# chanchanchan97/ICAFusion

Hardware: AMD Instinct MI355X
Metric: RGB/IR image-pairs/sec (two-stream forward + NMS) (higher is better)
Workload: dtype bf16

## Files before the change

icafusion_amd/csrc/cstream.hip:

```cpp
#include "conv_common.h"

namespace icaf {

constexpr int CS_C = 64, CS_TH = 8, CS_TW = 16, CS_HH = CS_TH + 2, CS_HWD = CS_TW + 2, CS_PITCH = 24;
constexpr int CS_NIDX = CS_HH * CS_PITCH;
constexpr int CS_PATCH = CS_NIDX * 128;
constexpr int CS_WBYTES = 9 * CS_C * 128;
constexpr int CS_W2BYTES = CS_C * 128;
constexpr int CS_SO = CS_C * 2 + 16;
constexpr int CS_STG = 128 * CS_SO;
constexpr int CS_LDS = CS_WBYTES + CS_W2BYTES + 2 * CS_PATCH + CS_STG;
static_assert(CS_LDS <= 160 * 1024, "LDS capacity");

struct CsGeom { int tiles_x, tiles_y, ntile; };

template <int DT, bool CHAIN>
__global__ __launch_bounds__(512) __attribute__((amdgpu_waves_per_eu(2, 2))) void cstream_kernel(const ConvP p, const CsGeom gm) {
    using E = Elem<DT>;
    static_assert(DT != ICAF_F32, "16-bit types");
    constexpr int RB = 128, NSTEP = 4, VEC = E::VEC;
    extern __shared__ __attribute__((aligned(1024))) unsigned char lds[];
    unsigned char* wbuf = lds;
    unsigned char* w2buf = lds + CS_WBYTES;
    unsigned char* patch0 = w2buf + CS_W2BYTES;
    unsigned char* stg = patch0 + 2 * CS_PATCH;

    const int tid = threadIdx.x, lane = tid & 63, l31 = lane & 31, hi = lane >> 5;
    const int wave = __builtin_amdgcn_readfirstlane(tid >> 6);
    const int g = blockIdx.z;
    const int wm = wave & 3, wn = wave >> 2;
    const int sy = wm >> 1, sx = wm & 1;

    const __amdgpu_buffer_rsrc_t xr = __builtin_amdgcn_make_buffer_rsrc(
        (void*)((const typename E::type*)p.x + g * p.x_gs), 0, p.x_bytes, 0x00020000);
    const __amdgpu_buffer_rsrc_t wr = __builtin_amdgcn_make_buffer_rsrc(
        (void*)((const typename E::type*)p.w + g * p.w_gs), 0, p.w_bytes, 0x00020000);
    constexpr unsigned OOB = 0x80000000u;

    {
        const int rsub = lane >> 3;
        for (int t = wave; t < 72; t += 8) {
            const int c = t >> 3, j = t & 7;
// ... 31 lines not shown
            const int hy = idx / CS_PITCH, hx = idx - hy * CS_PITCH;
            const int gy = y0 - 1 + hy, gx = x0 - 1 + hx;
            const bool ok = hx < CS_HWD && (unsigned)gy < (unsigned)p.H && (unsigned)gx < (unsigned)p.W;
            const unsigned voff = ok ? img_off + (unsigned)((gy * p.W + gx) * p.ldx) * E::BYTES + (unsigned)(cs << 4) : OOB;
            __builtin_amdgcn_raw_ptr_buffer_load_lds(xr, (lds_ptr_t)(dst + (j << 10)), 16, voff, 0, 0, 0);
        }
    };

    f32x4 bq[4], bq2[4];
    {
        const float* __restrict__ bias = p.bias ? p.bias + g * p.bias_gs : nullptr;
        const float* __restrict__ bias2 = (CHAIN && p.bias2) ? p.bias2 + g * p.bias2_gs : nullptr;
#pragma unroll
        for (int qd = 0; qd < 4; ++qd) {
            const int n = wn * 32 + 8 * qd + 4 * hi;
            const f32x4 t1 = *(const f32x4*)((bias && n < p.Cout) ? bias + n : (const float*)p.w);
            bq[qd] = (bias && n < p.Cout) ? t1 : f32x4{0.f, 0.f, 0.f, 0.f};
            const f32x4 t2 = *(const f32x4*)((bias2 && n < p.Cout2) ? bias2 + n : (const float*)p.w);
            bq2[qd] = (bias2 && n < p.Cout2) ? t2 : f32x4{0.f, 0.f, 0.f, 0.f};
        }
#pragma unroll
        for (int qd = 0; qd < 4; ++qd) asm volatile("" : "+v"(bq[qd]), "+v"(bq2[qd]));
    }
    const int fkey = (l31 >> 1) & 7;
    int foff[NSTEP];
#pragma unroll
    for (int s = 0; s < NSTEP; ++s) foff[s] = (wn * 32 + l31) * RB + (((2 * s + hi) ^ fkey) << 4);
    const int lpy = sy * 4 + (l31 >> 3), lpx = sx * 8 + (l31 & 7);
    const int lbase = lpy * CS_PITCH + lpx;
    const int srow = wm * 32 + l31;

    int t = t_lo + lb;
    if (t >= t_hi) { wait_vmcnt<0>(); return; }
    issue_patch(t, 0);

    typename E::type* __restrict__ yg = (typename E::type*)p.y + g * p.y_gs;
    const typename E::type* __restrict__ rg = p.res ? (const typename E::type*)p.res + g * p.res_gs : nullptr;
    typename E::type* __restrict__ y2g = CHAIN ? (typename E::type*)p.y2 + g * p.y2_gs : nullptr;
    const float alpha_acc = p.alpha_acc[g], alpha_res = p.alpha_res[g];

    auto row_to_m = [&](int r, int b, int y0, int x0) {
        const int st = r >> 5, q = r & 31;
        const int gy = y0 + (st >> 1) * 4 + (q >> 3), gx = x0 + (st & 1) * 8 + (q & 7);
        return (gy < p.Ho && gx < p.Wo) ? (b * p.Ho + gy) * p.Wo + gx : -1;
    };
    u32x4 rres[2] = {u32x4{0u, 0u, 0u, 0u}, u32x4{0u, 0u, 0u, 0u}};
    auto flush = [&](typename E::type* dst, int ldd, int cout, int b, int y0, int x0, bool rr) {
#pragma unroll
        for (int it = 0; it < 2; ++it) {
            const int idx = tid + it * 512, row = idx >> 3, cv = idx & 7;
            const int m = row_to_m(row, b, y0, x0), n = cv * VEC;
            if (m >= 0 && n < cout) {
                u32x4 sv = *(const u32x4*)(stg + row * CS_SO + cv * 16);
                if (rr) {
                    float v[VEC], r[VEC];
                    unpack16<DT>(sv, v);
                    unpack16<DT>(rres[it], r);
#pragma unroll
                    for (int j = 0; j < VEC; ++j) v[j] = __builtin_fmaf(alpha_res, r[j], v[j]);
                    sv = pack16<DT>(v);
                }
                *(u32x4*)(dst + (long long)m * ldd + n) = sv;
            }
        }
    };
    auto load_res = [&](int b, int y0, int x0) {
#pragma unroll
        for (int it = 0; it < 2; ++it) {
            const int idx = tid + it * 512, row = idx >> 3, cv = idx & 7;
            const int m = row_to_m(row, b, y0, x0);
            rres[it] = *(const u32x4*)(rg + (long long)(m < 0 ? 0 : m) * p.ldr + cv * VEC);
        }
    };
    auto stage = [&](const f32x16& acc, const f32x4 (&bv)[4], float scale) {
#pragma unroll
        for (int qd = 0; qd < 4; ++qd) {
            const int nl = wn * 32 + 8 * qd + 4 * hi;
            float v[4];
#pragma unroll
            for (int j = 0; j < 4; ++j) v[j] = acc[4 * qd + j] + bv[qd][j] + 0.0f;
            silu4_f(v, v);
#pragma unroll
            for (int j = 0; j < 4; ++j) v[j] *= scale;
            u32x2 pk;
            if constexpr (DT == ICAF_BF16) { pk[0] = pack2_bf16(v[0], v[1]); pk[1] = pack2_bf16(v[2], v[3]); }
            else { pk[0] = pack2_f16(v[0], v[1]); pk[1] = pack2_f16(v[2], v[3]); }
            *(u32x2*)(stg + srow * CS_SO + nl * E::BYTES) = pk;
        }
    };

    int cur = 0, pb = -1, py0 = 0, px0 = 0;
    while (true) {
        int b, y0, x0;
        decode(t, b, y0, x0);
        const int tn = t + wgx;
        wait_vmcnt<0>();
        asm volatile("s_waitcnt lgkmcnt(0)" ::: "memory");
        __builtin_amdgcn_s_barrier();
        if (pb >= 0) {
            if constexpr (CHAIN) flush(y2g, p.ldy2, p.Cout2, pb, py0, px0, false);
            else flush(yg, p.ldy, p.Cout, pb, py0, px0, rg != nullptr);
        }
        if (rg) load_res(b, y0, x0);
        if (tn < t_hi) issue_patch(tn, cur ^ 1);
        const unsigned char* patch = patch0 + cur * CS_PATCH;
        f32x16 acc;
#pragma unroll
        for (int r = 0; r < 16; ++r) acc[r] = 0.0f;
#pragma unroll
        for (int c = 0; c < 9; ++c) {
            const int ky = c / 3, kx = c - 3 * ky;
            const int idx = lbase + ky * CS_PITCH + kx;
            const unsigned char* pe = patch + (idx << 7);
            const int key = (idx >> 1) & 7;
#pragma unroll
            for (int s = 0; s < NSTEP; ++s) {
                const u32x4 fp = *(const u32x4*)(pe + (((2 * s + hi) ^ key) << 4));
                const u32x4 fw = *(const u32x4*)(wbuf + c * (CS_C * RB) + foff[s]);
                mma_step<DT>(acc, fw, fp);
            }
        }
        lds_barrier();
        stage(acc, bq, alpha_acc);
        pb = b; py0 = y0; px0 = x0;
        if constexpr (CHAIN) {
            lds_barrier();
            if (rg) { wait_vmcnt<0>(); }
#pragma unroll
            for (int it = 0; it < 2; ++it) {
                const int idx = tid + it * 512, row = idx >> 3, cv = idx & 7;
                const int m = row_to_m(row, b, y0, x0), n = cv * VEC;
                if (m >= 0 && n < p.Cout) {
                    u32x4 sv = *(const u32x4*)(stg + row * CS_SO + cv * 16);
                    if (rg) {
                        float v[VEC], r[VEC];
                        unpack16<DT>(sv, v);
                        unpack16<DT>(rres[it], r);
#pragma unroll
                        for (int j = 0; j < VEC; ++j) v[j] = __builtin_fmaf(alpha_res, r[j], v[j]);
                        sv = pack16<DT>(v);
                        *(u32x4*)(stg + row * CS_SO + cv * 16) = sv;
                    }
                    if (p.keep1) *(u32x4*)(yg + (long long)m * p.ldy + n) = sv;
                }
            }
            lds_barrier();
            f32x16 acc2;
#pragma unroll
            for (int r = 0; r < 16; ++r) acc2[r] = 0.0f;
#pragma unroll
            for (int s = 0; s < NSTEP; ++s) {
                const u32x4 fp2 = *(const u32x4*)(stg + srow * CS_SO + ((2 * s + hi) << 4));
                const u32x4 fw2 = *(const u32x4*)(w2buf + foff[s]);
                mma_step<DT>(acc2, fw2, fp2);
            }
            lds_barrier();
            stage(acc2, bq2, 1.0f);
        }
        if (tn >= t_hi) break;
        t = tn;
        cur ^= 1;
    }
    wait_vmcnt<0>();
    lds_barrier();
    if constexpr (CHAIN) flush(y2g, p.ldy2, p.Cout2, pb, py0, px0, false);
    else flush(yg, p.ldy, p.Cout, pb, py0, px0, rg != nullptr);
}

int cstream_check(const icaf_conv_args* a, const ConvP& p) {
    if (a->dtype == ICAF_F32 || a->out_dtype != a->dtype) return fail(ICAF_ERR_UNSUPPORTED, "cstream: 16-bit types, out dtype == dtype");
    if (a->kh != 3 || a->kw != 3 || a->sh != 1 || a->sw != 1 || a->ph != 1 || a->pw != 1) return fail(ICAF_ERR_UNSUPPORTED, "cstream: 3x3 / stride 1 / pad 1 layers");
    if (a->Cin != CS_C || a->Cout > CS_C || a->Cout % 8 || a->Kp != 9 * CS_C) return fail(ICAF_ERR_UNSUPPORTED, "cstream: built for 64 -> (<= 64) channels (Cin = %d, Cout = %d, Kp = %d)", a->Cin, a->Cout, a->Kp);
    if (a->act != ICAF_ACT_SILU || a->pre) return fail(ICAF_ERR_UNSUPPORTED, "cstream: SiLU layers without a pre-activation term");
    if (p.x_bytes == 0) return fail(ICAF_ERR_UNSUPPORTED, "cstream: operand exceeds the 2 GiB buffer-descriptor range");
    if (!p.vec_y || (a->res && !p.vec_r)) return fail(ICAF_ERR_UNSUPPORTED, "cstream: y / res must take 16-byte vectors");
    if (a->w2) {
        if (a->Cout2 > CS_C || a->Cout2 % 8 || a->Kp2 != CS_C || !p.vec_y2 || a->Cout != CS_C) return fail(ICAF_ERR_UNSUPPORTED, "cstream: chained 1x1 of 64 -> (<= 64) channels with Kp2 = 64");
        if (a->res && !a->chain_keep) return fail(ICAF_ERR_UNSUPPORTED, "cstream: a residual needs chain_keep");
        if (a->chain_keep && (a->alpha_acc[0] != 1.0f || a->alpha_acc[1] != 1.0f)) return fail(ICAF_ERR_UNSUPPORTED, "cstream: chain_keep with alpha_acc != 1");
    }
    return ICAF_OK;
}

template <int DT, bool CHAIN>
static int launch_cstream_cfg(const ConvP& p, int groups, hipStream_t s) {
    CsGeom gm;
    gm.tiles_x = (p.Wo + CS_TW - 1) / CS_TW;
    gm.tiles_y = (p.Ho + CS_TH - 1) / CS_TH;
    gm.ntile = p.B * gm.tiles_x * gm.tiles_y;
    int dev = 0, cus = 256;
    ICAF_HIP(hipGetDevice(&dev));
    ICAF_HIP(hipDeviceGetAttribute(&cus, hipDeviceAttributeMultiprocessorCount, dev));
    int grid = (cus / groups) & ~7;
    if (grid < 8) grid = 8;
    ICAF_LDS_OPTIN((cstream_kernel<DT, CHAIN>), CS_LDS);
    cstream_kernel<DT, CHAIN><<<dim3((unsigned)grid, 1, (unsigned)groups), dim3(512), CS_LDS, s>>>(p, gm);
    ICAF_LAUNCH_CHECK();
    return ICAF_OK;
}

int launch_cstream(const icaf_conv_args* a, const ConvP& p, hipStream_t s) {
    int st = cstream_check(a, p);
    if (st) return st;
    if (a->dtype == ICAF_BF16) return a->w2 ? launch_cstream_cfg<ICAF_BF16, true>(p, a->groups, s) : launch_cstream_cfg<ICAF_BF16, false>(p, a->groups, s);
    return a->w2 ? launch_cstream_cfg<ICAF_F16, true>(p, a->groups, s) : launch_cstream_cfg<ICAF_F16, false>(p, a->groups, s);
}

}
```

icafusion_amd/csrc/igemm.hip:

```cpp
#include "conv_common.h"

static_assert(sizeof(icaf_conv_args) == 312, "icaf_conv_args layout is mirrored by ctypes in icafusion_amd/_lib.py");
static_assert(sizeof(icaf_bneck_args) == 376, "icaf_bneck_args layout is mirrored by ctypes in icafusion_amd/_lib.py");

namespace icaf {

template <int DT, int ODT, int BM, int BN, int WM, int WN, int ACT, int RB, int NS, int MODE, bool PRE, bool CHAIN = false>
__global__ __launch_bounds__((BM / WM) * (BN / WN) * 64) void igemm_dma_kernel(const ConvP p) {
    using E = Elem<DT>;
    using L = TileLds<DT, ODT, BM, BN>;
    constexpr int VEC = E::VEC;
    constexpr int BK = RB / E::BYTES;
    constexpr int SPR = RB / 16;
    constexpr int RPI = 1024 / RB;
    constexpr int AI = BM / RPI, BI = BN / RPI;
    constexpr int NW = (BM / WM) * (BN / WN);
    constexpr int NA = AI / NW;
    constexpr int NBF = BI / NW, NBR = BI % NW;
    constexpr int NBMAX = NBF + (NBR ? 1 : 0);
    constexpr int TM = WM / 32, TN = WN / 32;
    constexpr int WAVES_M = BM / WM;
    constexpr int STAGE = (BM + BN) * RB;
    constexpr int NSTEP = RB / 32;
    static_assert(AI % NW == 0 && (NW == 4 || NW == 8), "tile shape");
// ... 348 lines not shown
int launch_ctile(const icaf_conv_args* a, const ConvP& p, int shape, hipStream_t s);
int launch_bneck(const icaf_conv_args* a, const ConvP& p, int shape, hipStream_t s);
const char* ctile_tag(int shape);
int stream_check(const icaf_conv_args* a, const ConvP& p, int shape);
int launch_stream(const icaf_conv_args* a, const ConvP& p, int shape, hipStream_t s);
const char* stream_tag(int shape);
int cstream_check(const icaf_conv_args* a, const ConvP& p);
int launch_cstream(const icaf_conv_args* a, const ConvP& p, hipStream_t s);
int cwide_check(const icaf_conv_args* a, const ConvP& p, int shape);
int launch_cwide(const icaf_conv_args* a, const ConvP& p, int shape, hipStream_t s);
const char* cwide_tag(int shape);
int wreg_check(const icaf_conv_args* a, const ConvP& p, int shape);
int launch_wreg(const icaf_conv_args* a, const ConvP& p, int shape, hipStream_t s);
const char* wreg_tag(int shape);

static int pick_tile(const icaf_conv_args* a, const ConvP& p) {
    const bool dma_ok = p.x_bytes != 0;
    if (a->tile > 40 && a->tile < 90) return a->tile;
    if (a->tile >= 1 && a->tile <= 34 && a->tile % 10 >= 1 && a->tile % 10 <= 4) {
        const int pipe = a->tile / 10;
        return (pipe != 1 && !dma_ok) ? a->tile % 10 + 10 : a->tile;
    }
    if (a->tile == 25 || a->tile == 26 || a->tile == 28 || a->tile == 29) return a->tile;
    if (a->x2) return 81;
    const bool f32 = a->dtype == ICAF_F32 || a->out_dtype == ICAF_F32;
    const int N = a->Cout;
    const long long M = p.M;
    auto blocks = [&](int t) { return ((M + kTiles[t - 1].bm - 1) / kTiles[t - 1].bm) * ((N + kTiles[t - 1].bn - 1) / kTiles[t - 1].bn) * a->groups; };
    int t;
    if (N > 64 && !f32) t = 1;
    else if (N > 32) t = 2;
    else t = 3;
    if (t == 1 && blocks(1) < 512 && blocks(2) > blocks(1)) t = 2;
    if (blocks(t) < 512 && blocks(4) > blocks(t)) t = 4;
    if (!dma_ok) return t + 10;
    const int eb = a->dtype == ICAF_F32 ? 4 : 2;
    if (a->w2) {
        const int c = a->Cout > a->Cout2 ? a->Cout : a->Cout2;
        const bool w128 = ((long long)a->Cin * eb) % 128 == 0;
        if (c <= 64) return w128 ? 22 : 2;
        return w128 ? 21 : 1;
    }
    if (a->pre) {
        if (t > 2) t = 2;
        return ((long long)a->Cin * eb) % 128 == 0 ? t + 20 : t;
    }
    return (long long)p.K * eb >= 256 ? t + 20 : t;
// ... 168 lines not shown
    p.Kp2 = a->Kp2; p.Cout2 = a->Cout2; p.ldy2 = a->ldy2; p.keep1 = a->chain_keep;
    p.vec_y2 = a->w2 && (a->ldy2 % vo == 0) && (((uintptr_t)a->y2 & 15) == 0) && ((a->y2_gs * yb) % 16 == 0);
    p.w2_bytes = a->w2 ? (unsigned)((((long long)a->Cout2 + 127) / 128 * 128) * a->Kp2 * eb) : 0;
}

int conv_prepare(const icaf_conv_args* a, ConvP& p) {
    int st = validate(a);
    if (st) return st;
    fill(a, p);
    return ICAF_OK;
}

}

using namespace icaf;

extern "C" int icaf_conv2d(const icaf_conv_args* a, icaf_stream_t s) {
    int st = validate(a);
    if (st) return st;
    ConvP p;
    fill(a, p);
    const int tile = pick_tile(a, p);
    hipStream_t hs = S(s);
    if (a->x2 && tile != 81 && tile != 82) return fail(ICAF_ERR_UNSUPPORTED, "icaf_conv2d: x2 (C3 tail) is built for launch configurations 81 / 82 only (tile %d)", tile);
    if (tile == 71) return launch_cstream(a, p, hs);
    if (tile > 80) return launch_cwide(a, p, tile - 80, hs);
    if (tile > 70) return fail(ICAF_ERR_ARG, "unknown tile id %d", tile);
    if (tile > 60) return launch_wreg(a, p, tile - 60, hs);
    if (tile > 50) return launch_stream(a, p, tile - 50, hs);
    if (tile > 40) return launch_ctile(a, p, tile - 40, hs);
    if (a->dtype == ICAF_BF16)
        return a->out_dtype == ICAF_F32 ? launch_tile<ICAF_BF16, ICAF_F32>(p, a->groups, tile, hs)
                                        : launch_tile<ICAF_BF16, ICAF_BF16>(p, a->groups, tile, hs);
    if (a->dtype == ICAF_F16)
        return a->out_dtype == ICAF_F32 ? launch_tile<ICAF_F16, ICAF_F32>(p, a->groups, tile, hs)
                                        : launch_tile<ICAF_F16, ICAF_F16>(p, a->groups, tile, hs);
    return launch_tile<ICAF_F32, ICAF_F32>(p, a->groups, tile, hs);
}

extern "C" int icaf_bottleneck(const icaf_bneck_args* b, icaf_stream_t s) {
    if (!b || !b->w1) return fail(ICAF_ERR_ARG, "icaf_bottleneck: null pointer");
    const icaf_conv_args* a = &b->conv;
    int st = validate(a);
    if (st) return st;
    const int eb = a->dtype == ICAF_F32 ? 4 : 2;
    if (b->Kp1 * eb != 128) return fail(ICAF_ERR_ARG, "icaf_bottleneck: the packed 1x1 weights must have 128-byte rows (Kp1 = %d)", b->Kp1);
    if (a->pre) return fail(ICAF_ERR_ARG, "icaf_bottleneck: no pre-activation term");
    if (a->x2) return fail(ICAF_ERR_ARG, "icaf_bottleneck: conv.x2 must be NULL (the block's cv2 half is icaf_bneck_args.x2)");
    if (a->x == a->y) return fail(ICAF_ERR_ARG, "icaf_bottleneck: in-place operation is not possible (neighbouring patches read x)");
    ConvP p;
    fill(a, p);
    p.w1 = b->w1; p.bias1 = b->bias1; p.w1_gs = b->w1_gs; p.bias1_gs = b->bias1_gs; p.Kp1 = b->Kp1;
    p.w1_bytes = (unsigned)((((long long)a->Cout + 127) / 128 * 128) * b->Kp1 * eb);
    p.x2 = b->x2; p.x2_gs = b->x2_gs; p.ldx2 = b->ldx2;
    return launch_bneck(a, p, b->shape, S(s));
}

extern "C" int icaf_conv2d_kernel_name(const icaf_conv_args* a, char* buf, int buf_len) {
    int st = validate(a);
    if (st) return st;
    ConvP p;
    fill(a, p);
    const int tile = pick_tile(a, p);
    if (a->x2 && tile != 81 && tile != 82) return fail(ICAF_ERR_UNSUPPORTED, "icaf_conv2d: x2 (C3 tail) is built for launch configurations 81 / 82 only (tile %d)", tile);
    static const char* dn[] = {"f32", "bf16", "f16"};
    if (tile == 71) {
        st = cstream_check(a, p);
        if (st) return st;
        snprintf(buf, buf_len, "cstream_%s_8x16n64", dn[a->dtype]);
        return ICAF_OK;
    }
    if (tile > 80) {
        st = cwide_check(a, p, tile - 80);
        if (st) return st;
        snprintf(buf, buf_len, "cwide_%s_%s", dn[a->dtype], cwide_tag(tile - 80));
        return ICAF_OK;
    }
    if (tile > 70) return fail(ICAF_ERR_ARG, "unknown tile id %d", tile);
    if (tile > 60) {
        st = wreg_check(a, p, tile - 60);
        if (st) return st;
        snprintf(buf, buf_len, "igemm_wreg_%s_%s", dn[a->dtype], wreg_tag(tile - 60));
        return ICAF_OK;
    }
    if (tile > 50) {
        st = stream_check(a, p, tile - 50);
        if (st) return st;
// ... 14 lines not shown
```

icafusion_amd/models/common.py:

```python
import math

import torch
import torch.nn as nn

from .. import ops
from ..options import OPT
from ..engine import ImageIn, Plan, concat_view, from_act, to_act

BN_EPS_DEFAULT = 1e-5


def autopad(k, p=None):
    if p is None:
        p = k // 2 if isinstance(k, int) else [v // 2 for v in k]
    return p


def _pair(v):
    return (v, v) if isinstance(v, int) else tuple(v)


def _module_dtype(m, fallback=torch.float32):
    forced = getattr(m, "compute_dtype", None)
    if forced is not None:
# ... 182 lines not shown
        ch = None
        if chain is not None:
            convs, twin_convs, y2 = chain[:3]
            keep = len(chain) > 3 and bool(chain[3])
            x2 = chain[4] if len(chain) > 4 else None
            n2 = sum(c.conv.out_channels for c in convs)

            def pack2():
                packs = []
                for row in ([convs] + ([twin_convs] if paired else [])):
                    ws, bs = zip(*(c.folded() for c in row))
                    w2p, kp2 = ops.pack_conv_weight(torch.cat(ws), plan.dtype)
                    packs.append((w2p, kp2, ops.pack_bias(torch.cat(bs), n2)))
                if not paired:
                    return packs[0]
                return (torch.stack([p[0] for p in packs]).contiguous(), packs[0][1], torch.stack([p[2] for p in packs]).contiguous())
            w2p, kp2, b2p = self._cached(("chain",) + key_tail + tuple(id(c) for c in convs), pack2)
            ch = dict(w=w2p, kp=kp2, bias=b2p, y=y2, cout=n2, keep=keep)
            if x2 is not None:
                ch["x2"] = x2
            if not keep:
                out = y2[..., :c2] if y2.shape[-1] >= c2 else plan.act(B, Ho, Wo, c2, pair=paired)
        plan.add(ops.conv2d(x, wp, kp, bp, out, kh, kw, sh, sw, ph, pw, c1, c2, self._act_code(), res=res,
                            name=f"conv{kh}x{kw}s{sh}" + (("+cv3" if ch.get("x2") is not None else "+1x1") if ch else ""), pre=pre_term, chain=ch,
                            pre_nearest=pre_nearest))
        return (out if ch["keep"] else y2) if ch else out

    fuse_stem2 = True

    def stem2_ok(self, plan, x, nxt, c3):
        k0, k1 = self.conv, getattr(nxt, "conv", None)
        if not (self.fuse_stem2 and self.fuse_stem and isinstance(x, ImageIn) and x.pair and isinstance(nxt, Conv)
                and plan.dtype in (torch.bfloat16, torch.float16) and (not x.u8 or x.c0 == 0)):
            return False
        _, _, H, W = x.shape
        return ((k0.kernel_size, k0.stride, _pair(k0.padding), k0.in_channels, k0.out_channels) == ((6, 6), (2, 2), (2, 2), 3, 32)
                and k0.groups == 1 and isinstance(self.act, nn.SiLU) and H % 2 == 0 and W % 2 == 0
                and (k1.kernel_size, k1.stride, _pair(k1.padding), k1.in_channels, k1.out_channels) == ((3, 3), (2, 2), (1, 1), 32, 64)
                and nxt.chain_ok(plan, c3) and 2 * c3.cv1.conv.out_channels == 64)

    def emit_stem2(self, plan, x, twin, nxt, nxt_twin, convs, twin_convs, y2):
        key_tail = (plan.dtype, plan.device, id(twin))

        def stack(packs):
            return (torch.stack([p[0] for p in packs]).contiguous(), packs[0][1], torch.stack([p[2] for p in packs]).contiguous())

        def pack_row(rows, transform, cin_pad):
# ... 14 lines not shown
        return y2

    chain_fuse = True

    def chain_ok(self, plan, c3):
        k, cv = self.conv, c3.cv1.conv
        n1, n2 = k.out_channels, 2 * cv.out_channels
        return (self.chain_fuse and plan.dtype in (torch.bfloat16, torch.float16) and isinstance(self.act, nn.SiLU)
                and hasattr(k, "kernel_size") and k.kernel_size == (3, 3) and k.groups == 1 and k.in_channels % 32 == 0
                and cv.kernel_size == (1, 1) and cv.stride == (1, 1) and cv.in_channels == n1
                and c3.cv2.conv.out_channels == cv.out_channels and isinstance(c3.cv1.act, nn.SiLU)
                and max(n1, n2) <= self.chain_max_width)

    chain_max_width = 128

    def chain_ok_1x1(self, plan, nxt):
        k, kn = self.conv, nxt.conv
        return (self.chain_fuse and plan.dtype in (torch.bfloat16, torch.float16) and isinstance(self.act, nn.SiLU)
                and isinstance(nxt.act, nn.SiLU) and k.kernel_size == (3, 3) and k.groups == 1 and k.in_channels % 64 == 0
                and kn.kernel_size == (1, 1) and kn.stride == (1, 1) and kn.groups == 1 and kn.in_channels == k.out_channels
                and max(k.out_channels, kn.out_channels) <= self.chain_max_width)

    chain_tail = OPT.c3_tail

    def chain_ok_tail(self, plan, cv3):
        k, k3 = self.conv, cv3.conv
        return (self.chain_tail and OPT.cwide and plan.dtype in (torch.bfloat16, torch.float16) and isinstance(self.act, nn.SiLU)
                and isinstance(cv3.act, nn.SiLU) and (k.kernel_size, k.stride, _pair(k.padding), k.groups) == ((3, 3), (1, 1), (1, 1), 1)
                and (k.in_channels, k.out_channels) == (128, 128) and k3.kernel_size == (1, 1) and k3.stride == (1, 1) and k3.groups == 1
                and _pair(k3.padding) == (0, 0) and k3.in_channels == 2 * k.out_channels and k3.out_channels == 256)


class Bottleneck(HipModule):

    def __init__(self, c1, c2, shortcut=True, g=1, e=0.5):
        super().__init__()
        c_ = int(c2 * e)
        self.cv1 = Conv(c1, c_, 1, 1)
        self.cv2 = Conv(c_, c2, 3, 1, g=g)
        self.add = shortcut and c1 == c2

    def emit(self, plan, x, out=None, twin=None):
        t = self.cv1.emit(plan, x, twin=twin.cv1 if twin is not None else None)
        return self.cv2.emit(plan, t, out=out, res=x if self.add else None,
                             twin=twin.cv2 if twin is not None else None)

    fuse = True
    fuse_widths = (32,)

    def fusable(self, plan, x):
        a, b = self.cv1.conv, self.cv2.conv
        c = a.in_channels
        return (self.fuse and plan.dtype in (torch.bfloat16, torch.float16) and c in self.fuse_widths
# ... 90 lines not shown
        else:
            self.cv1.emit(plan, x, out=cat[..., :2 * c_], twin=twin.cv1 if paired else None, also=(self.cv2,),
                          twin_also=(twin.cv2,) if paired else ())
        if tail3:
            if out is None:
                out = plan.act(B, H, W, k3.out_channels, pair=paired)
            return self.m[0].emit_fused(plan, cat[..., :c_], None, twin=twin.m[0] if paired else None,
                                        cv3=(self.cv3, twin.cv3 if paired else None, cat[..., c_:2 * c_], out))
        cur = 0
        t_next = None
        for j, blk in enumerate(self.m):
            a = cat[..., cur * c_:(cur + 1) * c_]
            tw = twin.m[j] if paired else None
            if fused[j]:
                cur = 2 - cur
                blk.emit_fused(plan, a, cat[..., cur * c_:(cur + 1) * c_], twin=tw)
                continue
            nxt = self.m[j + 1] if j + 1 < len(self.m) and not fused[j + 1] else None
            t = t_next if t_next is not None else blk.cv1.emit(plan, a, twin=tw.cv1 if paired else None)
            t_next, ch = None, None
            if nxt is not None and self.chain_bottlenecks and blk.cv2.chain_ok_1x1(plan, nxt.cv1):
                t_next = plan.act(B, H, W, nxt.cv1.conv.out_channels, pair=paired)
                ch = ((nxt.cv1,), (twin.m[j + 1].cv1,) if paired else None, t_next, True)
            if j == len(self.m) - 1 and cur == 0 and blk.cv2.chain_ok_tail(plan, self.cv3):
                if out is None:
                    out = plan.act(B, H, W, k3.out_channels, pair=paired)
                return blk.cv2.emit(plan, t, out=a, res=a if blk.add else None, twin=tw.cv2 if paired else None,
                                    chain=((self.cv3,), (twin.cv3,) if paired else None, out, False, cat[..., c_:2 * c_]))
            blk.cv2.emit(plan, t, out=a, res=a if blk.add else None, twin=tw.cv2 if paired else None, chain=ch)
        src = cat[..., :2 * c_] if cur == 0 else cat[..., c_:3 * c_]
        return self.cv3.emit(plan, src, out=out, twin=twin.cv3 if paired else None, swap_halves=cur != 0)


class SPPF(HipModule):

    def __init__(self, c1, c2, k=5):
        super().__init__()
        c_ = c1 // 2
        self.cv1 = Conv(c1, c_, 1, 1)
        self.cv2 = Conv(c_ * 4, c2, 1, 1)
        self.m = nn.MaxPool2d(kernel_size=k, stride=1, padding=k // 2)

    def emit(self, plan, x, out=None, twin=None):
        B, H, W = x.shape[-4:-1]
        c_ = self.cv1.conv.out_channels
        k = self.m.kernel_size if isinstance(self.m.kernel_size, int) else self.m.kernel_size[0]
        paired = twin is not None
# ... 414 lines not shown
```

icafusion_amd/ops.py:

```python
import ctypes as C
import weakref

import torch

from . import _lib
from .options import OPT
from ._lib import BneckArgs, ConvArgs, DmffArgs, Stem2Args, check, lib, F32, BF16, F16, ACT_NONE, ACT_SILU, ACT_GELU

_DT = {torch.float32: F32, torch.bfloat16: BF16, torch.float16: F16}
VEC = {torch.float32: 4, torch.bfloat16: 8, torch.float16: 8}
N_ALIGN = 128
K_ALIGN_BYTES = 128


def dtype_code(dt):
    try:
        return _DT[dt]
    except KeyError:
        raise _lib.IcafError(f"unsupported dtype {dt}; supported: float32, bfloat16, float16") from None


def k_align(dt):
    return K_ALIGN_BYTES // torch.empty((), dtype=dt).element_size()

# ... 196 lines not shown
    if (kh, kw, ph, pw) != (3, 3, 1, 1) or sh != sw or cout % 128:
        return []
    if sh == 1:
        return [81, 82] if (cin == 128 and cout == 128) else []
    if sh == 2:
        if cin == 64:
            return [83, 85]
        if cin == 128:
            return [84]
    return []


def _conv_signature(a):
    return (a.B * a.Ho * a.Wo, a.Cout, a.Cin, a.kh, a.kw, a.sh, a.sw, a.H, a.W, a.ldx, a.ldy, a.groups, a.dtype,
            a.out_dtype, a.act, bool(a.res), bool(a.pre) + a.pre_mode, a.Cout2 if a.w2 else 0, 2 if a.x2 else bool(a.chain_keep))


def conv_candidates(a):
    cands = []
    cs_ok = ((a.kh, a.kw, a.sh, a.sw, a.ph, a.pw) == (3, 3, 1, 1, 1, 1) and a.Cin == 64 and a.Cout <= 64 and a.Cout % 8 == 0 and a.dtype != F32
             and a.out_dtype == a.dtype and a.act == ACT_SILU and not a.pre and OPT.cstream)
    cw = (cwide_shapes(a.kh, a.kw, a.sh, a.sw, a.ph, a.pw, a.Cin, a.Cout)
          if (a.dtype != F32 and a.wf and a.out_dtype == a.dtype and a.act == ACT_SILU and not a.pre and OPT.cwide) else [])
    if a.w2 and a.x2:
        cands = ([82] if a.B * a.Ho * a.Wo < OPT.tail_8x16_minpix else [81, 82]) if OPT.cwide else []
    elif a.w2:
        t = 2 if max(a.Cout, a.Cout2) <= 64 else 1
        cands = [t, t + 20]
        if cw and a.Cout == 128 and a.Cout2 <= 128 and a.Cout2 % 32 == 0:
            cands += cw
        if cs_ok and a.Cout == 64 and a.Cout2 <= 64:
            cands.append(71)
    elif a.pre:
        cands = [t + 10 * pipe for pipe in (0, 2) for t in (1, 2) if not (t == 1 and (a.out_dtype == F32 or a.Cout <= 64))]
        if a.dtype != F32 and a.out_dtype == a.dtype and a.Cout >= 128 and (a.Cin * 2) % 128 == 0:
            cands.append(28)
        if (a.dtype != F32 and a.out_dtype == a.dtype and (a.Cin * 2) % 128 == 0 and a.Cout % 8 == 0 and OPT.stream_gemm and a.act == ACT_SILU
                and (a.kh, a.kw, a.sh, a.sw, a.ph, a.pw) == (1, 1, 1, 1, 0, 0) and a.groups == 1):
            cands.append(52)
            if a.Cout > 64:
                cands.append(51)
    for pipe in (() if (a.pre or a.w2) else CONV_PIPELINES):
        for t in (1, 2, 3, 4):
            if t == 1 and (a.out_dtype == F32 or a.Cout <= 64):
                continue
            if t == 3 and a.Cout > 32:
                continue
# ... 550 lines not shown
```

icafusion_amd/options.py:

```python
import dataclasses
import os
from dataclasses import dataclass, field


def _f(default, env, doc, lib=False):
    return field(default=default, metadata={"env": env, "doc": doc, "lib": lib})


@dataclass
class PlanOptions:
    cwide: bool = _f(True, "ICAF_CWIDE", "resident-patch / streamed-weights 3x3 kernels (cwide.hip) as tuner candidates")
    cstream: bool = _f(True, "ICAF_CSTREAM", "persistent resident-filter 3x3 kernel (cstream.hip) as a tuner candidate")
    wreg_gemm: bool = _f(True, "ICAF_WREG_GEMM", "weights-from-registers GEMM kernels (igemm_wreg.hip) as tuner candidates")
    stream_gemm: bool = _f(True, "ICAF_STREAM_GEMM", "persistent streaming 1x1 kernel (igemm_stream.hip) as a tuner candidate")
    wreg64_maxpix: int = _f(128 * 1024, "ICAF_WREG64_MAXPIX", "launches with at most this many pixels are offered the 64-pixel wreg tiles")
    tail_8x16_minpix: int = _f(200_000, "ICAF_TAIL_8X16_MINPIX", "C3 tails with fewer pixels per stream are offered only the 8 x 8 cwide form")
    retune_tiles: frozenset = _f(frozenset(), "ICAF_RETUNE_TILES", "launch configurations that get their chance against a cached choice (e.g. 63:64)")
    retune_pre: bool = _f(False, "ICAF_RETUNE_PRE", "every configuration of the pre-activation-term launches is re-timed against the cached one")
    c3_tail: bool = _f(True, "ICAF_C3_TAIL", "a C3's cv3 rides on its last Bottleneck's 3x3 launch")
    dmff_fuse: bool = _f(True, "ICAF_DMFF_FUSE", "fused DMFF block launches (two / three per iteration) instead of seven per-layer launches")
    dmff_fuse_max_c: int = _f(64, "ICAF_DMFF_FUSE_MAX_C", "largest C the two-launch block kernel (dmff_fused.hip) takes")
    dmff_fuse_fp32: bool = _f(False, "ICAF_DMFF_FUSE_FP32", "fp32 plans also use the fused block kernels (their fp32 instantiations)")
    dmff_wide: bool = _f(True, "ICAF_DMFF_WIDE", "three-launch block kernels (dmff_wide.hip)")
    dmff_wide_max_c: int = _f(512, "ICAF_DMFF_WIDE_MAX_C", "largest C the three-launch block kernels take")
    dmff_res32: bool = _f(True, "ICAF_DMFF_RES32", "loops > 1: the token stream between iterations in fp32")
    detect_fuse: bool = _f(True, "ICAF_DETECT_FUSE", "Detect's 1x1 conv and the decode in one launch")
    dmff_qkv_npass: int = _f(0, "ICAF_DMFF_QKV_NPASS", "output-channel passes per workgroup of the wide LN + QKV kernel (0 = automatic)")
    dmff_ksplit: int = _f(0, "ICAF_DMFF_KSPLIT", "hidden-column split of the wide out-proj + MLP kernel (0 = automatic, 1 = never, 2 / 4 = force)")
    pipe_extra_plans: int = _f(1, "ICAF_PIPE_EXTRA_PLANS", "further sets of `depth` plans a host-fed pipeline owns (copy targets not in flight)")
    pipe_copy_streams: int = _f(1, "ICAF_PIPE_COPY_STREAMS", "a batch's host -> device copy in this many slices, one copy stream each")
    pipe_copy_prio: int = _f(-1, "ICAF_PIPE_COPY_PRIO", "priority of the copy stream(s): -1 = high (a hardware queue of their own)")
    pipe_branches: bool = _f(False, "ICAF_PIPE_BRANCHES", "host-fed pipelines keep the hipGraph's parallel branches (measured slower)")
    detect_elementwise: bool = _f(False, "ICAF_DETECT_ELEMENTWISE", "Detect decode by the one-thread-per-element kernel", lib=True)
    attn_qsplit: int = _f(0, "ICAF_ATTN_QSPLIT", "query splits per head of the attention kernel (0 = automatic)", lib=True)
    sppf_vpb: int = _f(0, "ICAF_SPPF_VPB", "channel vectors per workgroup of the SPPF kernel (0 = automatic)", lib=True)

    @staticmethod
    def _parse(f, text):
        t = f.type if isinstance(f.type, type) else {"bool": bool, "int": int, "frozenset": frozenset}[str(f.type)]
        if t is bool:
            return text.strip().lower() not in ("0", "", "false", "no", "off")
        if t is int:
# ... 37 lines not shown
```

Measured before the change: 17170.

## Fuse C3 cv3 1x1 tail into 64-channel cstream Bottleneck 3x3 kernel

Adds a TAIL mode to the 64-channel cstream 3x3 conv kernel. After the 3x3 conv, residual and SiLU, the kernel concatenates the result with the C3's cv1 branch (x2) in LDS and runs the cv3 1x1 (128 -> 128) in the same launch. Each half of the output is staged in a separate buffer, one of them reusing the spare patch buffer. This removes a separate cv3 launch and the round trip of the intermediate tensor through global memory for the 80x80 C3 blocks. In exchange it adds register pressure from the preloaded cv3 weights and extra barriers per tile, and it only applies when a map has at least the minimum pixel count.

```diff
diff --git a/icafusion_amd/csrc/cstream.hip b/icafusion_amd/csrc/cstream.hip
--- a/icafusion_amd/csrc/cstream.hip
+++ b/icafusion_amd/csrc/cstream.hip
@@ -11,13 +11,16 @@
 constexpr int CS_STG = 128 * CS_SO;
 constexpr int CS_LDS = CS_WBYTES + CS_W2BYTES + 2 * CS_PATCH + CS_STG;
 static_assert(CS_LDS <= 160 * 1024, "LDS capacity");
+constexpr int CS_TAIL_C2 = 2 * CS_C;
+static_assert(CS_STG <= CS_PATCH, "C3 tail: a 64-channel staging tile fits in a patch buffer");
 
 struct CsGeom { int tiles_x, tiles_y, ntile; };
 
-template <int DT, bool CHAIN>
+template <int DT, int CH>
 __global__ __launch_bounds__(512) __attribute__((amdgpu_waves_per_eu(2, 2))) void cstream_kernel(const ConvP p, const CsGeom gm) {
     using E = Elem<DT>;
     static_assert(DT != ICAF_F32, "16-bit types");
+    constexpr bool CHAIN = CH == 1, TAIL = CH == 2;
     constexpr int RB = 128, NSTEP = 4, VEC = E::VEC;
     extern __shared__ __attribute__((aligned(1024))) unsigned char lds[];
     unsigned char* wbuf = lds;
@@ -95,6 +98,24 @@
 #pragma unroll
         for (int qd = 0; qd < 4; ++qd) asm volatile("" : "+v"(bq[qd]), "+v"(bq2[qd]));
     }
+    u32x4 w3f[TAIL ? 2 : 1][TAIL ? 8 : 1];
+    f32x4 b3[TAIL ? 2 : 1][4];
+    if constexpr (TAIL) {
+        const typename E::type* __restrict__ w3g = (const typename E::type*)p.w2 + g * p.w2_gs;
+        const float* __restrict__ bias3 = p.bias2 ? p.bias2 + g * p.bias2_gs : nullptr;
+#pragma unroll
+        for (int pz = 0; pz < 2; ++pz) {
+            const int row = (wn + 2 * pz) * 32 + l31;
+#pragma unroll
+            for (int s = 0; s < 8; ++s) w3f[pz][s] = *(const u32x4*)(w3g + (long long)row * p.Kp2 + 16 * s + 8 * hi);
+#pragma unroll
+            for (int qd = 0; qd < 4; ++qd) {
+                const int n = pz * CS_C + wn * 32 + 8 * qd + 4 * hi;
+                const f32x4 t3 = *(const f32x4*)((bias3 && n < p.Cout2) ? bias3 + n : (const float*)p.w);
+                b3[pz][qd] = (bias3 && n < p.Cout2) ? t3 : f32x4{0.f, 0.f, 0.f, 0.f};
+            }
+        }
+    }
     const int fkey = (l31 >> 1) & 7;
     int foff[NSTEP];
 #pragma unroll
@@ -109,7 +130,8 @@
 
     typename E::type* __restrict__ yg = (typename E::type*)p.y + g * p.y_gs;
     const typename E::type* __restrict__ rg = p.res ? (const typename E::type*)p.res + g * p.res_gs : nullptr;
-    typename E::type* __restrict__ y2g = CHAIN ? (typename E::type*)p.y2 + g * p.y2_gs : nullptr;
+    typename E::type* __restrict__ y2g = (CHAIN || TAIL) ? (typename E::type*)p.y2 + g * p.y2_gs : nullptr;
+    const typename E::type* __restrict__ x2g = TAIL ? (const typename E::type*)p.x2 + g * p.x2_gs : nullptr;
     const float alpha_acc = p.alpha_acc[g], alpha_res = p.alpha_res[g];
 
     auto row_to_m = [&](int r, int b, int y0, int x0) {
@@ -118,13 +140,13 @@
         return (gy < p.Ho && gx < p.Wo) ? (b * p.Ho + gy) * p.Wo + gx : -1;
     };
     u32x4 rres[2] = {u32x4{0u, 0u, 0u, 0u}, u32x4{0u, 0u, 0u, 0u}};
-    auto flush = [&](typename E::type* dst, int ldd, int cout, int b, int y0, int x0, bool rr) {
+    auto flush = [&](const unsigned char* src, typename E::type* dst, int ldd, int n0, int cout, int b, int y0, int x0, bool rr) {
 #pragma unroll
         for (int it = 0; it < 2; ++it) {
             const int idx = tid + it * 512, row = idx >> 3, cv = idx & 7;
-            const int m = row_to_m(row, b, y0, x0), n = cv * VEC;
+            const int m = row_to_m(row, b, y0, x0), n = n0 + cv * VEC;
             if (m >= 0 && n < cout) {
-                u32x4 sv = *(const u32x4*)(stg + row * CS_SO + cv * 16);
+                u32x4 sv = *(const u32x4*)(src + row * CS_SO + cv * 16);
                 if (rr) {
                     float v[VEC], r[VEC];
                     unpack16<DT>(sv, v);
@@ -145,7 +167,7 @@
             rres[it] = *(const u32x4*)(rg + (long long)(m < 0 ? 0 : m) * p.ldr + cv * VEC);
         }
     };
-    auto stage = [&](const f32x16& acc, const f32x4 (&bv)[4], float scale) {
+    auto stage = [&](unsigned char* dst, const f32x16& acc, const f32x4 (&bv)[4], float scale) {
 #pragma unroll
         for (int qd = 0; qd < 4; ++qd) {
             const int nl = wn * 32 + 8 * qd + 4 * hi;
@@ -158,7 +180,16 @@
             u32x2 pk;
             if constexpr (DT == ICAF_BF16) { pk[0] = pack2_bf16(v[0], v[1]); pk[1] = pack2_bf16(v[2], v[3]); }
             else { pk[0] = pack2_f16(v[0], v[1]); pk[1] = pack2_f16(v[2], v[3]); }
-            *(u32x2*)(stg + srow * CS_SO + nl * E::BYTES) = pk;
+            *(u32x2*)(dst + srow * CS_SO + nl * E::BYTES) = pk;
+        }
+    };
+    u32x4 xcat[TAIL ? 2 : 1];
+    auto load_x2 = [&](int b, int y0, int x0) {
+#pragma unroll
+        for (int it = 0; it < 2; ++it) {
+            const int idx = tid + it * 512, row = idx >> 3, cv = idx & 7;
+            const int m = row_to_m(row, b, y0, x0);
+            xcat[it] = *(const u32x4*)(x2g + (long long)(m < 0 ? 0 : m) * p.ldx2 + cv * VEC);
         }
     };
 
@@ -171,10 +202,15 @@
         asm volatile("s_waitcnt lgkmcnt(0)" ::: "memory");
         __builtin_amdgcn_s_barrier();
         if (pb >= 0) {
-            if constexpr (CHAIN) flush(y2g, p.ldy2, p.Cout2, pb, py0, px0, false);
-            else flush(yg, p.ldy, p.Cout, pb, py0, px0, rg != nullptr);
+            if constexpr (TAIL) {
+                flush(stg, y2g, p.ldy2, 0, p.Cout2, pb, py0, px0, false);
+                flush(patch0 + (cur ^ 1) * CS_PATCH, y2g, p.ldy2, CS_C, p.Cout2, pb, py0, px0, false);
+                lds_barrier();
+            } else if constexpr (CHAIN) flush(stg, y2g, p.ldy2, 0, p.Cout2, pb, py0, px0, false);
+            else flush(stg, yg, p.ldy, 0, p.Cout, pb, py0, px0, rg != nullptr);
         }
         if (rg) load_res(b, y0, x0);
+        if constexpr (TAIL) load_x2(b, y0, x0);
         if (tn < t_hi) issue_patch(tn, cur ^ 1);
         const unsigned char* patch = patch0 + cur * CS_PATCH;
         f32x16 acc;
@@ -194,8 +230,41 @@
             }
         }
         lds_barrier();
-        stage(acc, bq, alpha_acc);
+        stage(stg, acc, bq, alpha_acc);
         pb = b; py0 = y0; px0 = x0;
+        if constexpr (TAIL) {
+            unsigned char* c2buf = patch0 + cur * CS_PATCH;
+            lds_barrier();
+            wait_vmcnt<0>();
+#pragma unroll
+            for (int it = 0; it < 2; ++it) {
+                const int idx = tid + it * 512, row = idx >> 3, cv = idx & 7;
+                if (rg) {
+                    float v[VEC], r[VEC];
+                    unpack16<DT>(*(const u32x4*)(stg + row * CS_SO + cv * 16), v);
+                    unpack16<DT>(rres[it], r);
+#pragma unroll
+                    for (int j = 0; j < VEC; ++j) v[j] = __builtin_fmaf(alpha_res, r[j], v[j]);
+                    *(u32x4*)(stg + row * CS_SO + cv * 16) = pack16<DT>(v);
+                }
+                *(u32x4*)(c2buf + row * CS_SO + cv * 16) = xcat[it];
+            }
+            lds_barrier();
+            f32x16 acc3[2];
+#pragma unroll
+            for (int pz = 0; pz < 2; ++pz)
+#pragma unroll
+                for (int r = 0; r < 16; ++r) acc3[pz][r] = 0.0f;
+#pragma unroll
+            for (int s = 0; s < 8; ++s) {
+                const u32x4 fp3 = *(const u32x4*)((s < 4 ? stg : c2buf) + srow * CS_SO + ((2 * (s & 3) + hi) << 4));
+#pragma unroll
+                for (int pz = 0; pz < 2; ++pz) mma_step<DT>(acc3[pz], w3f[pz][s], fp3);
+            }
+            lds_barrier();
+            stage(stg, acc3[0], b3[0], 1.0f);
+            stage(c2buf, acc3[1], b3[1], 1.0f);
+        }
         if constexpr (CHAIN) {
             lds_barrier();
             if (rg) { wait_vmcnt<0>(); }
@@ -228,7 +297,7 @@
                 mma_step<DT>(acc2, fw2, fp2);
             }
             lds_barrier();
-            stage(acc2, bq2, 1.0f);
+            stage(stg, acc2, bq2, 1.0f);
         }
         if (tn >= t_hi) break;
         t = tn;
@@ -236,8 +305,11 @@
     }
     wait_vmcnt<0>();
     lds_barrier();
-    if constexpr (CHAIN) flush(y2g, p.ldy2, p.Cout2, pb, py0, px0, false);
-    else flush(yg, p.ldy, p.Cout, pb, py0, px0, rg != nullptr);
+    if constexpr (TAIL) {
+        flush(stg, y2g, p.ldy2, 0, p.Cout2, pb, py0, px0, false);
+        flush(patch0 + cur * CS_PATCH, y2g, p.ldy2, CS_C, p.Cout2, pb, py0, px0, false);
+    } else if constexpr (CHAIN) flush(stg, y2g, p.ldy2, 0, p.Cout2, pb, py0, px0, false);
+    else flush(stg, yg, p.ldy, 0, p.Cout, pb, py0, px0, rg != nullptr);
 }
 
 int cstream_check(const icaf_conv_args* a, const ConvP& p) {
@@ -247,7 +319,13 @@
     if (a->act != ICAF_ACT_SILU || a->pre) return fail(ICAF_ERR_UNSUPPORTED, "cstream: SiLU layers without a pre-activation term");
     if (p.x_bytes == 0) return fail(ICAF_ERR_UNSUPPORTED, "cstream: operand exceeds the 2 GiB buffer-descriptor range");
     if (!p.vec_y || (a->res && !p.vec_r)) return fail(ICAF_ERR_UNSUPPORTED, "cstream: y / res must take 16-byte vectors");
-    if (a->w2) {
+    if (a->x2) {
+        if (!a->w2) return fail(ICAF_ERR_ARG, "cstream: x2 without the chained layer's weights (w2)");
+        if (a->Cout != CS_C || a->Cout2 != CS_TAIL_C2 || a->Kp2 != CS_TAIL_C2 || !p.vec_y2)
+            return fail(ICAF_ERR_UNSUPPORTED, "cstream: the C3 tail is a 1x1 of [64 | 64] -> 128 channels with Kp2 = 128 (Cout = %d, Cout2 = %d, Kp2 = %d)", a->Cout, a->Cout2, a->Kp2);
+        if (a->ldx2 < CS_C || a->ldx2 % 8 || ((uintptr_t)a->x2 & 15) || (a->x2_gs * 2) % 16) return fail(ICAF_ERR_ARG, "cstream: x2 must take 16-byte vectors (ldx2 = %d)", a->ldx2);
+        if (a->chain_keep) return fail(ICAF_ERR_UNSUPPORTED, "cstream: the C3 tail does not keep the intermediate tensor");
+    } else if (a->w2) {
         if (a->Cout2 > CS_C || a->Cout2 % 8 || a->Kp2 != CS_C || !p.vec_y2 || a->Cout != CS_C) return fail(ICAF_ERR_UNSUPPORTED, "cstream: chained 1x1 of 64 -> (<= 64) channels with Kp2 = 64");
         if (a->res && !a->chain_keep) return fail(ICAF_ERR_UNSUPPORTED, "cstream: a residual needs chain_keep");
         if (a->chain_keep && (a->alpha_acc[0] != 1.0f || a->alpha_acc[1] != 1.0f)) return fail(ICAF_ERR_UNSUPPORTED, "cstream: chain_keep with alpha_acc != 1");
@@ -255,7 +333,7 @@
     return ICAF_OK;
 }
 
-template <int DT, bool CHAIN>
+template <int DT, int CH>
 static int launch_cstream_cfg(const ConvP& p, int groups, hipStream_t s) {
     CsGeom gm;
     gm.tiles_x = (p.Wo + CS_TW - 1) / CS_TW;
@@ -266,8 +344,8 @@
     ICAF_HIP(hipDeviceGetAttribute(&cus, hipDeviceAttributeMultiprocessorCount, dev));
     int grid = (cus / groups) & ~7;
     if (grid < 8) grid = 8;
-    ICAF_LDS_OPTIN((cstream_kernel<DT, CHAIN>), CS_LDS);
-    cstream_kernel<DT, CHAIN><<<dim3((unsigned)grid, 1, (unsigned)groups), dim3(512), CS_LDS, s>>>(p, gm);
+    ICAF_LDS_OPTIN((cstream_kernel<DT, CH>), CS_LDS);
+    cstream_kernel<DT, CH><<<dim3((unsigned)grid, 1, (unsigned)groups), dim3(512), CS_LDS, s>>>(p, gm);
     ICAF_LAUNCH_CHECK();
     return ICAF_OK;
 }
@@ -275,8 +353,10 @@
 int launch_cstream(const icaf_conv_args* a, const ConvP& p, hipStream_t s) {
     int st = cstream_check(a, p);
     if (st) return st;
-    if (a->dtype == ICAF_BF16) return a->w2 ? launch_cstream_cfg<ICAF_BF16, true>(p, a->groups, s) : launch_cstream_cfg<ICAF_BF16, false>(p, a->groups, s);
-    return a->w2 ? launch_cstream_cfg<ICAF_F16, true>(p, a->groups, s) : launch_cstream_cfg<ICAF_F16, false>(p, a->groups, s);
-}
-
-}
+    const int ch = a->x2 ? 2 : a->w2 ? 1 : 0;
+    if (a->dtype == ICAF_BF16)
+        return ch == 2 ? launch_cstream_cfg<ICAF_BF16, 2>(p, a->groups, s) : ch ? launch_cstream_cfg<ICAF_BF16, 1>(p, a->groups, s) : launch_cstream_cfg<ICAF_BF16, 0>(p, a->groups, s);
+    return ch == 2 ? launch_cstream_cfg<ICAF_F16, 2>(p, a->groups, s) : ch ? launch_cstream_cfg<ICAF_F16, 1>(p, a->groups, s) : launch_cstream_cfg<ICAF_F16, 0>(p, a->groups, s);
+}
+
+}
diff --git a/icafusion_amd/csrc/igemm.hip b/icafusion_amd/csrc/igemm.hip
--- a/icafusion_amd/csrc/igemm.hip
+++ b/icafusion_amd/csrc/igemm.hip
@@ -394,7 +394,7 @@
         return (pipe != 1 && !dma_ok) ? a->tile % 10 + 10 : a->tile;
     }
     if (a->tile == 25 || a->tile == 26 || a->tile == 28 || a->tile == 29) return a->tile;
-    if (a->x2) return 81;
+    if (a->x2) return a->Cin == 64 ? 71 : 81;
     const bool f32 = a->dtype == ICAF_F32 || a->out_dtype == ICAF_F32;
     const int N = a->Cout;
     const long long M = p.M;
@@ -609,7 +609,7 @@
     fill(a, p);
     const int tile = pick_tile(a, p);
     hipStream_t hs = S(s);
-    if (a->x2 && tile != 81 && tile != 82) return fail(ICAF_ERR_UNSUPPORTED, "icaf_conv2d: x2 (C3 tail) is built for launch configurations 81 / 82 only (tile %d)", tile);
+    if (a->x2 && tile != 71 && tile != 81 && tile != 82) return fail(ICAF_ERR_UNSUPPORTED, "icaf_conv2d: x2 (C3 tail) is built for launch configurations 71 / 81 / 82 only (tile %d)", tile);
     if (tile == 71) return launch_cstream(a, p, hs);
     if (tile > 80) return launch_cwide(a, p, tile - 80, hs);
     if (tile > 70) return fail(ICAF_ERR_ARG, "unknown tile id %d", tile);
@@ -649,7 +649,7 @@
     ConvP p;
     fill(a, p);
     const int tile = pick_tile(a, p);
-    if (a->x2 && tile != 81 && tile != 82) return fail(ICAF_ERR_UNSUPPORTED, "icaf_conv2d: x2 (C3 tail) is built for launch configurations 81 / 82 only (tile %d)", tile);
+    if (a->x2 && tile != 71 && tile != 81 && tile != 82) return fail(ICAF_ERR_UNSUPPORTED, "icaf_conv2d: x2 (C3 tail) is built for launch configurations 71 / 81 / 82 only (tile %d)", tile);
     static const char* dn[] = {"f32", "bf16", "f16"};
     if (tile == 71) {
         st = cstream_check(a, p);
diff --git a/icafusion_amd/models/common.py b/icafusion_amd/models/common.py
--- a/icafusion_amd/models/common.py
+++ b/icafusion_amd/models/common.py
@@ -228,7 +228,8 @@
             if not keep:
                 out = y2[..., :c2] if y2.shape[-1] >= c2 else plan.act(B, Ho, Wo, c2, pair=paired)
         plan.add(ops.conv2d(x, wp, kp, bp, out, kh, kw, sh, sw, ph, pw, c1, c2, self._act_code(), res=res,
-                            name=f"conv{kh}x{kw}s{sh}" + (("+cv3" if ch.get("x2") is not None else "+1x1") if ch else ""), pre=pre_term, chain=ch,
+                            name=f"conv{kh}x{kw}s{sh}" + ((("+cv3" + ("c64" if c2 == 64 else "")) if ch.get("x2") is not None else "+1x1") if ch else ""),
+                            pre=pre_term, chain=ch,
                             pre_nearest=pre_nearest))
         return (out if ch["keep"] else y2) if ch else out
 
@@ -289,13 +290,21 @@
                 and max(k.out_channels, kn.out_channels) <= self.chain_max_width)
 
     chain_tail = OPT.c3_tail
-
-    def chain_ok_tail(self, plan, cv3):
+    chain_tail64 = OPT.c3_tail64
+    chain_tail64_minpix = OPT.tail64_minpix
+
+    def chain_ok_tail(self, plan, cv3, pixels):
         k, k3 = self.conv, cv3.conv
-        return (self.chain_tail and OPT.cwide and plan.dtype in (torch.bfloat16, torch.float16) and isinstance(self.act, nn.SiLU)
-                and isinstance(cv3.act, nn.SiLU) and (k.kernel_size, k.stride, _pair(k.padding), k.groups) == ((3, 3), (1, 1), (1, 1), 1)
-                and (k.in_channels, k.out_channels) == (128, 128) and k3.kernel_size == (1, 1) and k3.stride == (1, 1) and k3.groups == 1
-                and _pair(k3.padding) == (0, 0) and k3.in_channels == 2 * k.out_channels and k3.out_channels == 256)
+        if not (plan.dtype in (torch.bfloat16, torch.float16) and isinstance(self.act, nn.SiLU) and isinstance(cv3.act, nn.SiLU)
+                and (k.kernel_size, k.stride, _pair(k.padding), k.groups) == ((3, 3), (1, 1), (1, 1), 1)
+                and k3.kernel_size == (1, 1) and k3.stride == (1, 1) and k3.groups == 1 and _pair(k3.padding) == (0, 0)
+                and k3.in_channels == 2 * k.out_channels):
+            return False
+        if (k.in_channels, k.out_channels) == (128, 128):
+            return self.chain_tail and OPT.cwide and k3.out_channels == 256
+        if (k.in_channels, k.out_channels) == (64, 64):
+            return self.chain_tail64 and OPT.cstream and k3.out_channels == 128 and pixels >= self.chain_tail64_minpix
+        return False
 
 
 class Bottleneck(HipModule):
@@ -432,7 +441,7 @@
             if nxt is not None and self.chain_bottlenecks and blk.cv2.chain_ok_1x1(plan, nxt.cv1):
                 t_next = plan.act(B, H, W, nxt.cv1.conv.out_channels, pair=paired)
                 ch = ((nxt.cv1,), (twin.m[j + 1].cv1,) if paired else None, t_next, True)
-            if j == len(self.m) - 1 and cur == 0 and blk.cv2.chain_ok_tail(plan, self.cv3):
+            if j == len(self.m) - 1 and cur == 0 and blk.cv2.chain_ok_tail(plan, self.cv3, B * H * W):
                 if out is None:
                     out = plan.act(B, H, W, k3.out_channels, pair=paired)
                 return blk.cv2.emit(plan, t, out=a, res=a if blk.add else None, twin=tw.cv2 if paired else None,
diff --git a/icafusion_amd/ops.py b/icafusion_amd/ops.py
--- a/icafusion_amd/ops.py
+++ b/icafusion_amd/ops.py
@@ -242,7 +242,9 @@
              and a.out_dtype == a.dtype and a.act == ACT_SILU and not a.pre and OPT.cstream)
     cw = (cwide_shapes(a.kh, a.kw, a.sh, a.sw, a.ph, a.pw, a.Cin, a.Cout)
           if (a.dtype != F32 and a.wf and a.out_dtype == a.dtype and a.act == ACT_SILU and not a.pre and OPT.cwide) else [])
-    if a.w2 and a.x2:
+    if a.w2 and a.x2 and a.Cin == 64:
+        cands = [71] if (cs_ok and a.Cout == 64 and a.Cout2 == 128) else []
+    elif a.w2 and a.x2:
         cands = ([82] if a.B * a.Ho * a.Wo < OPT.tail_8x16_minpix else [81, 82]) if OPT.cwide else []
     elif a.w2:
         t = 2 if max(a.Cout, a.Cout2) <= 64 else 1
diff --git a/icafusion_amd/options.py b/icafusion_amd/options.py
--- a/icafusion_amd/options.py
+++ b/icafusion_amd/options.py
@@ -18,6 +18,8 @@
     retune_tiles: frozenset = _f(frozenset(), "ICAF_RETUNE_TILES", "launch configurations that get their chance against a cached choice (e.g. 63:64)")
     retune_pre: bool = _f(False, "ICAF_RETUNE_PRE", "every configuration of the pre-activation-term launches is re-timed against the cached one")
     c3_tail: bool = _f(True, "ICAF_C3_TAIL", "a C3's cv3 rides on its last Bottleneck's 3x3 launch")
+    c3_tail64: bool = _f(True, "ICAF_C3_TAIL64", "... and so does it for 64-channel Bottlenecks (cstream.hip's C3 tail: the 80 x 80 blocks of yolov5s)")
+    tail64_minpix: int = _f(6_400, "ICAF_TAIL64_MINPIX", "64-channel C3 tails are used on maps with at least this many pixels per stream (one 80 x 80 map)")
     dmff_fuse: bool = _f(True, "ICAF_DMFF_FUSE", "fused DMFF block launches (two / three per iteration) instead of seven per-layer launches")
     dmff_fuse_max_c: int = _f(64, "ICAF_DMFF_FUSE_MAX_C", "largest C the two-launch block kernel (dmff_fused.hip) takes")
     dmff_fuse_fp32: bool = _f(False, "ICAF_DMFF_FUSE_FP32", "fp32 plans also use the fused block kernels (their fp32 instantiations)")
```

Result: no change. 17300 (median of 6 runs) (+0.8%).
